# haoheliu/AudioLDM2

Hardware: NVIDIA H100
Metric: 10s clips/sec @200 DDIM steps (audioldm2-full) (higher is better)
Workload: dtype f16x2 (split-fp16 tensor-core operands: weights hi + lo, activations hi + lo in the convolutions and one plane on the token side; fp32 accumulate, fp32 residual stream)

## Files before the change

### audioldm2_b200/csrc/attention.cu

```cuda
#include <float.h>
#include <stdlib.h>

#include "common.cuh"

namespace aldm {

static constexpr int ATT_D = 32;

__device__ __forceinline__ float ex2_approx(float x) {
  float y;
  asm("ex2.approx.ftz.f32 %0, %1;" : "=f"(y) : "f"(x));
  return y;
}

__device__ __forceinline__ void store_out_row(const aldm_attn_desc& d, long long orow, int h, const float* o) {
  aldm_plane_t* hp = reinterpret_cast<aldm_plane_t*>(d.out_hi) + orow * d.ldo + h * ATT_D;
  aldm_plane_t* lp = d.out_lo ? reinterpret_cast<aldm_plane_t*>(d.out_lo) + orow * d.ldo + h * ATT_D : nullptr;
#pragma unroll
  for (int i = 0; i < ATT_D; i += 8) {
    uint4 hh, ll;
    split8(o + i, hh, ll);
    *reinterpret_cast<uint4*>(hp + i) = hh;
    if (lp) *reinterpret_cast<uint4*>(lp + i) = ll;
  }
}

namespace atc {
constexpr int QT = 128, KT = 64, NS = 4;
constexpr int QA = 0;
constexpr int KB = QA + QT * 128;
constexpr int VT = KB + NS * KT * 128;
constexpr int BAR = VT + NS * ATT_D * 128;
constexpr int SMEM = BAR + 128 + 1024;
}

__device__ __forceinline__ uint32_t pack_half2(float a, float b) {
  const __half2 h = __floats2half2_rn(a, b);
  return *reinterpret_cast<const uint32_t*>(&h);
}

__global__ void __launch_bounds__(288, 2) attention_tc_kernel(const __grid_constant__ aldm_attn_desc d) {
  using namespace atc;
  extern __shared__ uint8_t smem_raw[];
  const uint32_t raw = smem_u32(smem_raw);
  const uint32_t base = (raw + 1023u) & ~1023u;
  const uint32_t bar = base + BAR;
  const uint32_t q_full = bar, kv_full0 = bar + 8, kv_empty0 = kv_full0 + 8 * NS;
  const int tid = threadIdx.x, warp = tid >> 5, lane = tid & 31;
  const int b = blockIdx.z, h = blockIdx.y, q0 = blockIdx.x * QT;
  const int bkv = d.kv_bmod > 0 ? b % d.kv_bmod : b;
  const int nt = (d.Nk + KT - 1) / KT;

  if (tid == 0) {
    mbar_init(q_full, 32);
    for (int i = 0; i < NS; ++i) { mbar_init(kv_full0 + 8 * i, 32); mbar_init(kv_empty0 + 8 * i, 8); }
    fence_barrier_init();
  }
  __syncthreads();
  pdl_wait();

  if (warp < 8) {
    const int wg = warp >> 2, g = lane >> 2, t = lane & 3;
    const int rloc = wg * 64 + (warp & 3) * 16 + g;
    const float sl2 = d.scale * 1.4426950408889634f;
    const float* mrow = d.mask ? d.mask + (long long)bkv * d.Nk : nullptr;
    const uint64_t dQ = wgmma_desc_sw128(base + QA + wg * 64 * 128);
    float o[16];
#pragma unroll
    for (int i = 0; i < 16; ++i) o[i] = 0.f;
    float mrun[2] = {-INFINITY, -INFINITY}, lrun[2] = {0.f, 0.f};
    mbar_wait(q_full, 0);
    for (int it = 0; it < nt; ++it) {
      const int k0 = it * KT, st = it % NS;
      mbar_wait(kv_full0 + 8 * st, (it / NS) & 1);
      fence_proxy_async();
      float s[32];
#pragma unroll
      for (int i = 0; i < 32; ++i) s[i] = 0.f;
      const uint64_t dK = wgmma_desc_sw128(base + KB + st * (KT * 128));
      wgmma_fence();
#pragma unroll
      for (int ks = 0; ks < 2; ++ks) wgmma_ss<KT>(s, dQ + 2 * ks, dK + 2 * ks, 1);
      wgmma_commit();
      wgmma_wait<0>();
      wgmma_fence_regs<32>(s);
      float mnew[2], corr[2];
      if (k0 + KT <= d.Nk && !mrow) {
#pragma unroll
        for (int hr = 0; hr < 2; ++hr) {
          float tmax = s[2 * hr];
#pragma unroll
          for (int j = 0; j < 8; ++j) tmax = fmaxf(tmax, fmaxf(s[4 * j + 2 * hr], s[4 * j + 2 * hr + 1]));
          tmax = fmaxf(tmax, __shfl_xor_sync(0xffffffffu, tmax, 1));
          tmax = fmaxf(tmax, __shfl_xor_sync(0xffffffffu, tmax, 2));
          mnew[hr] = fmaxf(mrun[hr], tmax * sl2);
          corr[hr] = ex2_approx(mrun[hr] - mnew[hr]);
#pragma unroll
          for (int j = 0; j < 8; ++j)
#pragma unroll
            for (int e = 0; e < 2; ++e) s[4 * j + 2 * hr + e] = ex2_approx(fmaf(s[4 * j + 2 * hr + e], sl2, -mnew[hr]));
        }
      } else {
#pragma unroll
        for (int hr = 0; hr < 2; ++hr) {
          float tmax = -INFINITY;
#pragma unroll
          for (int j = 0; j < 8; ++j)
#pragma unroll
            for (int e = 0; e < 2; ++e) {
              const int key = k0 + 8 * j + 2 * t + e;
              float v = s[4 * j + 2 * hr + e] * sl2;
              if (key >= d.Nk) v = -INFINITY;
              else if (mrow && __ldg(mrow + key) != 1.0f) v = -FLT_MAX;
              s[4 * j + 2 * hr + e] = v;
              tmax = fmaxf(tmax, v);
            }
          tmax = fmaxf(tmax, __shfl_xor_sync(0xffffffffu, tmax, 1));
          tmax = fmaxf(tmax, __shfl_xor_sync(0xffffffffu, tmax, 2));
          mnew[hr] = fmaxf(mrun[hr], tmax);
          corr[hr] = (mrun[hr] == -INFINITY) ? 0.f : ex2_approx(mrun[hr] - mnew[hr]);
#pragma unroll
          for (int j = 0; j < 8; ++j)
#pragma unroll
            for (int e = 0; e < 2; ++e) {
              const float v = s[4 * j + 2 * hr + e];
              s[4 * j + 2 * hr + e] = (v == -INFINITY) ? 0.f : ex2_approx(v - mnew[hr]);
            }
        }
      }
#pragma unroll
      for (int hr = 0; hr < 2; ++hr) {
        float ps = 0.f;
#pragma unroll
        for (int j = 0; j < 8; ++j) ps += s[4 * j + 2 * hr] + s[4 * j + 2 * hr + 1];
        lrun[hr] = lrun[hr] * corr[hr] + ps;
        mrun[hr] = mnew[hr];
#pragma unroll
        for (int j = 0; j < 4; ++j) { o[4 * j + 2 * hr] *= corr[hr]; o[4 * j + 2 * hr + 1] *= corr[hr]; }
      }
      uint32_t pa[4][4];
#pragma unroll
      for (int kc = 0; kc < 4; ++kc) {
        pa[kc][0] = pack_half2(s[8 * kc + 0], s[8 * kc + 1]);
        pa[kc][1] = pack_half2(s[8 * kc + 2], s[8 * kc + 3]);
        pa[kc][2] = pack_half2(s[8 * kc + 4], s[8 * kc + 5]);
        pa[kc][3] = pack_half2(s[8 * kc + 6], s[8 * kc + 7]);
      }
      const uint64_t dV = wgmma_desc_sw128(base + VT + st * (ATT_D * 128));
      wgmma_fence();
#pragma unroll
      for (int kc = 0; kc < 4; ++kc) wgmma_rs<ATT_D>(o, pa[kc], dV + 2 * kc, 1);
      wgmma_commit();
      wgmma_wait<0>();
      wgmma_fence_regs<16>(o);
      __syncwarp();
      if (lane == 0) mbar_arrive(kv_empty0 + 8 * st);
    }
    if (tid == 0) pdl_launch();
#pragma unroll
    for (int hr = 0; hr < 2; ++hr) {
      float l = lrun[hr];
      l += __shfl_xor_sync(0xffffffffu, l, 1);
      l += __shfl_xor_sync(0xffffffffu, l, 2);
      const int q = q0 + rloc + 8 * hr;
      if (q < d.Nq) {
        const float inv = 1.0f / l;
        const long long orow = (long long)b * d.Nq + q;
        aldm_plane_t* hp = reinterpret_cast<aldm_plane_t*>(d.out_hi) + orow * d.ldo + h * ATT_D + 2 * t;
        aldm_plane_t* lp = d.out_lo ? reinterpret_cast<aldm_plane_t*>(d.out_lo) + orow * d.ldo + h * ATT_D + 2 * t : nullptr;
#pragma unroll
        for (int j = 0; j < 4; ++j) {
          uint32_t hh, ll;
          split2(o[4 * j + 2 * hr] * inv, o[4 * j + 2 * hr + 1] * inv, hh, ll);
          *reinterpret_cast<uint32_t*>(hp + 8 * j) = hh;
          if (lp) *reinterpret_cast<uint32_t*>(lp + 8 * j) = ll;
        }
      }
    }
  } else {
    const aldm_plane_t* qh = reinterpret_cast<const aldm_plane_t*>(d.q_hi);
    const aldm_plane_t* kh = reinterpret_cast<const aldm_plane_t*>(d.k_hi);
    const aldm_plane_t* vh = reinterpret_cast<const aldm_plane_t*>(d.vt_hi);
    for (int idx = lane; idx < QT * 4; idx += 32) {
      const int r = idx >> 2, c = idx & 3;
      const bool ok = q0 + r < d.Nq;
      const long long off = ok ? ((long long)b * d.Nq + q0 + r) * d.ldq + d.q_col + h * ATT_D + c * 8 : 0;
      cp_async_16(base + QA + r * 128 + ((uint32_t)(c ^ (r & 7)) << 4), qh + off, ok ? 16u : 0u);
    }
    cp_async_mbar_arrive_noinc(q_full);
    const int ck = lane & 3, rk = lane >> 2;
    const int cv = lane & 7, rv = lane >> 3;
    const aldm_plane_t* kcol = kh + (long long)bkv * d.Nk * d.ldk + d.k_col + h * ATT_D + ck * 8;
    const long long vrow0 = ((long long)(bkv * d.heads + h) * ATT_D + rv) * d.ld_t + cv * 8;
    const long long kstep = 8ll * d.ldk, vstep = 4ll * d.ld_t;
    for (int it = 0, s = 0, ph = 1; it < nt; ++it) {
      const int k0 = it * KT;
      mbar_wait(kv_empty0 + 8 * s, ph);
      const uint32_t kb = base + KB + s * (KT * 128);
      const aldm_plane_t* kp = kcol + (long long)(k0 + rk) * d.ldk;
#pragma unroll
      for (int i = 0; i < KT / 8; ++i) {
        const int r = rk + 8 * i;
        const bool ok = k0 + r < d.Nk;
        cp_async_16(kb + r * 128 + ((uint32_t)(ck ^ (r & 7)) << 4), ok ? kp + i * kstep : kcol, ok ? 16u : 0u);
      }
      const uint32_t vb = base + VT + s * (ATT_D * 128);
      const bool vok = k0 + cv * 8 < d.Nk;
#pragma unroll
      for (int i = 0; i < ATT_D / 4; ++i) {
        const int r = rv + 4 * i;
        const aldm_plane_t* vp = vh + vrow0 + i * vstep + k0;
        cp_async_16(vb + r * 128 + ((uint32_t)(cv ^ (r & 7)) << 4), vok ? vp : vh, vok ? 16u : 0u);
      }
      cp_async_mbar_arrive_noinc(kv_full0 + 8 * s);
      if (++s == NS) { s = 0; ph ^= 1; }
    }
  }
}

template <int NKT>
__global__ void __launch_bounds__(128) attention_short_kernel(const __grid_constant__ aldm_attn_desc d) {
  __shared__ __align__(16) float sk[NKT][ATT_D];
  __shared__ __align__(16) float sv[NKT][ATT_D];
  __shared__ int sstate[NKT];
  const int tid = threadIdx.x;
  const int b = blockIdx.z, h = blockIdx.y;
  const int bkv = d.kv_bmod > 0 ? b % d.kv_bmod : b;
  pdl_wait();
  {
    const aldm_plane_t* kh = reinterpret_cast<const aldm_plane_t*>(d.k_hi);
    const aldm_plane_t* vh = reinterpret_cast<const aldm_plane_t*>(d.vt_hi);
    for (int idx = tid; idx < NKT * ATT_D; idx += 128) {
      const int key = idx / ATT_D, dim = idx % ATT_D;
      float kv = 0.f, vv = 0.f;
      if (key < d.Nk) {
        const long long ki = ((long long)bkv * d.Nk + key) * d.ldk + d.k_col + h * ATT_D + dim;
        const long long vi = ((long long)(bkv * d.heads + h) * ATT_D + dim) * d.ld_t + key;
        kv = plane_to_f(kh[ki]);
        vv = plane_to_f(vh[vi]);
      }
      sk[key][dim] = kv;
      sv[key][dim] = vv;
    }
    if (tid < NKT) sstate[tid] = tid >= d.Nk ? 2 : ((d.mask && __ldg(d.mask + (long long)bkv * d.Nk + tid) != 1.0f) ? 1 : 0);
  }
  __syncthreads();
  pdl_launch();
  const int q = blockIdx.x * 128 + tid;
  if (q >= d.Nq) return;
  float qv[ATT_D];
  {
    const long long qi = ((long long)b * d.Nq + q) * d.ldq + d.q_col + h * ATT_D;
    const uint4* ph = reinterpret_cast<const uint4*>(reinterpret_cast<const aldm_plane_t*>(d.q_hi) + qi);
#pragma unroll
    for (int c = 0; c < 4; ++c) {
      const uint4 a = __ldg(ph + c);
      const uint32_t aw[4] = {a.x, a.y, a.z, a.w};
#pragma unroll
      for (int e = 0; e < 4; ++e) {
        const float2 f = unpack2(aw[e]);
        qv[c * 8 + 2 * e] = f.x;
        qv[c * 8 + 2 * e + 1] = f.y;
      }
    }
  }
  const float sl2 = d.scale * 1.4426950408889634f;
  float sc[NKT];
  float mx = -INFINITY;
#pragma unroll
  for (int k = 0; k < NKT; ++k) {
    float acc = 0.f;
#pragma unroll
    for (int dd = 0; dd < ATT_D; dd += 4) {
      const float4 kk = *reinterpret_cast<const float4*>(&sk[k][dd]);
      acc = fmaf(qv[dd], kk.x, acc); acc = fmaf(qv[dd + 1], kk.y, acc);
      acc = fmaf(qv[dd + 2], kk.z, acc); acc = fmaf(qv[dd + 3], kk.w, acc);
    }
    const int st = sstate[k];
    const float v = st == 0 ? acc * sl2 : (st == 1 ? -FLT_MAX : -INFINITY);
    sc[k] = v;
    mx = fmaxf(mx, v);
  }
  float l = 0.f;
#pragma unroll
  for (int k = 0; k < NKT; ++k) {
    const float pk = sc[k] == -INFINITY ? 0.f : ex2_approx(sc[k] - mx);
    sc[k] = pk;
    l += pk;
  }
  float o[ATT_D];
#pragma unroll
  for (int i = 0; i < ATT_D; ++i) o[i] = 0.f;
#pragma unroll
  for (int k = 0; k < NKT; ++k) {
#pragma unroll
    for (int dd = 0; dd < ATT_D; dd += 4) {
      const float4 vv = *reinterpret_cast<const float4*>(&sv[k][dd]);
      o[dd] = fmaf(sc[k], vv.x, o[dd]); o[dd + 1] = fmaf(sc[k], vv.y, o[dd + 1]);
      o[dd + 2] = fmaf(sc[k], vv.z, o[dd + 2]); o[dd + 3] = fmaf(sc[k], vv.w, o[dd + 3]);
    }
  }
  const float inv = 1.0f / l;
#pragma unroll
  for (int i = 0; i < ATT_D; ++i) o[i] *= inv;
  store_out_row(d, (long long)b * d.Nq + q, h, o);
}

__global__ void __launch_bounds__(128) attention_simt_kernel(const __grid_constant__ aldm_attn_desc d) {
  const int b = blockIdx.z, h = blockIdx.y;
  const int qi = blockIdx.x * blockDim.x + threadIdx.x;
  if (qi >= d.Nq) return;
  const int bkv = d.kv_bmod > 0 ? b % d.kv_bmod : b;
  auto ld = [](const void* hi, const void* , long long i) {
    return plane_to_f(reinterpret_cast<const aldm_plane_t*>(hi)[i]);
  };
  float q[ATT_D], o[ATT_D];
  for (int i = 0; i < ATT_D; ++i) {
    q[i] = ld(d.q_hi, d.q_lo, ((long long)b * d.Nq + qi) * d.ldq + d.q_col + h * ATT_D + i) * d.scale;
    o[i] = 0.f;
  }
  float mrun = -INFINITY, lrun = 0.f;
  for (int k = 0; k < d.Nk; ++k) {
    float s = 0.f;
    const long long kr = ((long long)bkv * d.Nk + k) * d.ldk + d.k_col + h * ATT_D;
    for (int i = 0; i < ATT_D; ++i) s = fmaf(q[i], ld(d.k_hi, d.k_lo, kr + i), s);
    if (d.mask && d.mask[(long long)bkv * d.Nk + k] != 1.0f) s = -FLT_MAX;
    const float mnew = fmaxf(mrun, s);
    const float corr = (mrun == -INFINITY) ? 0.f : expf(mrun - mnew);
    const float p = expf(s - mnew);
    lrun = lrun * corr + p;
    for (int i = 0; i < ATT_D; ++i)
      o[i] = o[i] * corr + p * ld(d.vt_hi, d.vt_lo, ((long long)(bkv * d.heads + h) * ATT_D + i) * d.ld_t + k);
    mrun = mnew;
  }
  for (int i = 0; i < ATT_D; ++i) o[i] /= lrun;
  store_out_row(d, (long long)b * d.Nq + qi, h, o);
}

int attention_launch(const aldm_attn_desc& d, cudaStream_t st) {
  ALDM_REQUIRE(d.q_hi && d.k_hi && d.vt_hi && d.out_hi, ALDM_E_ARG, "attention: null pointer");
  ALDM_REQUIRE(d.B > 0 && d.heads > 0 && d.Nq > 0 && d.Nk > 0, ALDM_E_SHAPE, "attention: B=%d heads=%d Nq=%d Nk=%d", d.B,
               d.heads, d.Nq, d.Nk);
  ALDM_REQUIRE(d.ldq % 8 == 0 && d.ldk % 8 == 0 && d.ld_t % 8 == 0 && d.ldo % 8 == 0 && d.q_col % 8 == 0 && d.k_col % 8 == 0,
               ALDM_E_ALIGN, "attention: leading dims / column offsets must be multiples of 8");
  ALDM_REQUIRE(d.ld_t >= d.Nk, ALDM_E_SHAPE, "attention: ld_t=%d < Nk=%d", d.ld_t, d.Nk);
  ALDM_REQUIRE(aligned16(d.q_hi) && aligned16(d.k_hi) && aligned16(d.vt_hi) && aligned16(d.out_hi) && aligned16(d.out_lo),
               ALDM_E_ALIGN, "attention: pointers must be 16B aligned");
  ALDM_REQUIRE(d.heads <= 65535 && d.B <= 65535, ALDM_E_SHAPE, "attention: grid too large");
  if (d.impl == ALDM_GEMM_SIMT) {
    dim3 grid(cdiv(d.Nq, 128), d.heads, d.B);
    attention_simt_kernel<<<grid, 128, 0, st>>>(d);
  } else if (d.Nk <= 32 && !(getenv("ALDM_ATTN_SHORT") && getenv("ALDM_ATTN_SHORT")[0] == '0')) {
    dim3 grid(cdiv(d.Nq, 128), d.heads, d.B);
    if (d.Nk <= 8) ALDM_CHECK_CUDA(launch_pdl(attention_short_kernel<8>, grid, dim3(128), 0, st, d));
    else if (d.Nk <= 16) ALDM_CHECK_CUDA(launch_pdl(attention_short_kernel<16>, grid, dim3(128), 0, st, d));
    else ALDM_CHECK_CUDA(launch_pdl(attention_short_kernel<32>, grid, dim3(128), 0, st, d));
  } else {
    static bool configured = false;
    if (!configured) {
      ALDM_CHECK_CUDA(cudaFuncSetAttribute(attention_tc_kernel, cudaFuncAttributeMaxDynamicSharedMemorySize, atc::SMEM));
      configured = true;
    }
    dim3 grid(cdiv(d.Nq, atc::QT), d.heads, d.B);
    ALDM_CHECK_CUDA(launch_pdl(attention_tc_kernel, grid, dim3(288), atc::SMEM, st, d));
  }
  ALDM_CHECK_CUDA(cudaGetLastError());
  return ALDM_OK;
}

__global__ void softmax_rows_kernel(const float* __restrict__ x, int n, float scale, aldm_plane_t* __restrict__ hi,
                                    aldm_plane_t* __restrict__ lo) {
  __shared__ float red[32];
  const long long row = blockIdx.x;
  const float* xp = x + row * n;
  float mx = -INFINITY;
  for (int i = threadIdx.x; i < n; i += blockDim.x) mx = fmaxf(mx, xp[i] * scale);
  for (int o = 16; o > 0; o >>= 1) mx = fmaxf(mx, __shfl_xor_sync(0xffffffffu, mx, o));
  if ((threadIdx.x & 31) == 0) red[threadIdx.x >> 5] = mx;
  __syncthreads();
  mx = red[0];
  for (int w = 1; w < (blockDim.x >> 5); ++w) mx = fmaxf(mx, red[w]);
  __syncthreads();
  float s = 0.f;
  for (int i = threadIdx.x; i < n; i += blockDim.x) s += expf(xp[i] * scale - mx);
  for (int o = 16; o > 0; o >>= 1) s += __shfl_xor_sync(0xffffffffu, s, o);
  if ((threadIdx.x & 31) == 0) red[threadIdx.x >> 5] = s;
  __syncthreads();
  s = 0.f;
  for (int w = 0; w < (blockDim.x >> 5); ++w) s += red[w];
  const float inv = 1.0f / s;
  for (int i = threadIdx.x * 2; i < n; i += blockDim.x * 2) {
    const float a = expf(xp[i] * scale - mx) * inv;
    const float b = (i + 1 < n) ? expf(xp[i + 1] * scale - mx) * inv : 0.f;
    uint32_t h, l;
    split2(a, b, h, l);
    if (i + 1 < n) {
      *reinterpret_cast<uint32_t*>(hi + row * n + i) = h;
      if (lo) *reinterpret_cast<uint32_t*>(lo + row * n + i) = l;
    } else {
      store_split1(hi, lo, row * n + i, a);
    }
  }
}

}

extern "C" int aldm_attention(const aldm_attn_desc* d, void* stream) {
  if (!d) { aldm::set_error("aldm_attention: null desc"); return ALDM_E_ARG; }
  return aldm::attention_launch(*d, reinterpret_cast<cudaStream_t>(stream));
}

extern "C" int aldm_softmax_rows(const float* x, int32_t rows, int32_t n, float scale, void* out_hi, void* out_lo,
                                 void* stream) {
  using namespace aldm;
  ALDM_REQUIRE(x && out_hi && rows > 0 && n > 0, ALDM_E_ARG, "softmax_rows: bad arguments");
  ALDM_REQUIRE(n % 2 == 0, ALDM_E_UNSUPPORTED, "softmax_rows: n must be even");
  softmax_rows_kernel<<<rows, 256, 0, reinterpret_cast<cudaStream_t>(stream)>>>(
      x, n, scale, reinterpret_cast<aldm_plane_t*>(out_hi), reinterpret_cast<aldm_plane_t*>(out_lo));
  ALDM_CHECK_CUDA(cudaGetLastError());
  return ALDM_OK;
}
```

Before: 1.852.

## Pipeline QK and PV wgmma in attention, add lazy rescale and small-Nq config

Restructures the tensor-core attention loop so the QK^T wgmma for the next key tile is issued together with the PV wgmma of the current tile, and softmax runs while PV is in flight. Adds conditional rescaling: the running max is only raised when it grows by more than a threshold, so the output rescale is skipped warp-wide when no row changed. Adds a compile-time PLAIN variant with no mask or tail handling, and a one-warpgroup config for small Nq. This trades more register pressure and extra template instantiations for fewer serialized tensor-core waits. The lazy max also lets exponent values exceed 1 by up to 2^8, which adds fp16 range risk in P.

```diff
diff --git a/audioldm2_b200/csrc/attention.cu b/audioldm2_b200/csrc/attention.cu
--- a/audioldm2_b200/csrc/attention.cu
+++ b/audioldm2_b200/csrc/attention.cu
@@ -26,12 +26,19 @@
 }
 
 namespace atc {
-constexpr int QT = 128, KT = 64, NS = 4;
-constexpr int QA = 0;
-constexpr int KB = QA + QT * 128;
-constexpr int VT = KB + NS * KT * 128;
-constexpr int BAR = VT + NS * ATT_D * 128;
-constexpr int SMEM = BAR + 128 + 1024;
+constexpr int KT = 64, NS = 4;
+constexpr float TAU = 8.f;
+template <int NWG>
+struct Cfg {
+  static constexpr int QT = 64 * NWG;
+  static constexpr int THREADS = 128 * NWG + 32;
+  static constexpr int QA = 0;
+  static constexpr int KB = QA + QT * 128;
+  static constexpr int VT = KB + NS * KT * 128;
+  static constexpr int BAR = VT + NS * ATT_D * 128;
+  static constexpr int SMEM = BAR + 128 + 1024;
+  static constexpr int MIN_CTAS = NWG == 2 ? 2 : 3;
+};
 }
 
 __device__ __forceinline__ uint32_t pack_half2(float a, float b) {
@@ -39,123 +46,174 @@
   return *reinterpret_cast<const uint32_t*>(&h);
 }
 
-__global__ void __launch_bounds__(288, 2) attention_tc_kernel(const __grid_constant__ aldm_attn_desc d) {
+__device__ __forceinline__ void fence_regs_u32(uint32_t (&a)[4][4]) {
+#pragma unroll
+  for (int i = 0; i < 4; ++i)
+#pragma unroll
+    for (int j = 0; j < 4; ++j) asm volatile("" : "+r"(a[i][j])::"memory");
+}
+
+template <bool PLAIN>
+__device__ __forceinline__ void softmax_tile(float (&s)[32], int k0, int t, int Nk, const float* mrow, float sl2,
+                                             float (&mrun)[2], float (&lrun)[2], float (&corr)[2]) {
   using namespace atc;
+  const bool plain = PLAIN || (k0 + KT <= Nk && !mrow);
+  uint32_t out = 0, off = 0;
+  if (!plain) {
+#pragma unroll
+    for (int i = 0; i < 16; ++i) {
+      const int key = k0 + 8 * (i >> 1) + 2 * t + (i & 1);
+      if (key >= Nk) out |= 1u << i;
+      else if (mrow && __ldg(mrow + key) != 1.0f) off |= 1u << i;
+    }
+  }
+  float tmax[2];
+#pragma unroll
+  for (int hr = 0; hr < 2; ++hr) {
+    float m = -INFINITY;
+    if (plain) {
+#pragma unroll
+      for (int j = 0; j < 8; ++j) m = fmaxf(m, fmaxf(s[4 * j + 2 * hr], s[4 * j + 2 * hr + 1]));
+    } else {
+#pragma unroll
+      for (int j = 0; j < 8; ++j)
+#pragma unroll
+        for (int e = 0; e < 2; ++e) {
+          const uint32_t bit = 1u << (2 * j + e);
+          float v = s[4 * j + 2 * hr + e] * sl2;
+          if (out & bit) v = -INFINITY;
+          else if (off & bit) v = -FLT_MAX;
+          s[4 * j + 2 * hr + e] = v;
+          m = fmaxf(m, v);
+        }
+    }
+    m = fmaxf(m, __shfl_xor_sync(0xffffffffu, m, 1));
+    m = fmaxf(m, __shfl_xor_sync(0xffffffffu, m, 2));
+    tmax[hr] = plain ? m * sl2 : m;
+  }
+#pragma unroll
+  for (int hr = 0; hr < 2; ++hr) {
+    corr[hr] = 1.f;
+    if (tmax[hr] > mrun[hr] + TAU) {
+      corr[hr] = ex2_approx(mrun[hr] - tmax[hr]);
+      mrun[hr] = tmax[hr];
+    }
+    const float m = mrun[hr];
+    float ps = 0.f;
+    if (plain) {
+#pragma unroll
+      for (int j = 0; j < 8; ++j)
+#pragma unroll
+        for (int e = 0; e < 2; ++e) {
+          float& v = s[4 * j + 2 * hr + e];
+          v = ex2_approx(fmaf(v, sl2, -m));
+          ps += v;
+        }
+    } else {
+#pragma unroll
+      for (int j = 0; j < 8; ++j)
+#pragma unroll
+        for (int e = 0; e < 2; ++e) {
+          float& v = s[4 * j + 2 * hr + e];
+          v = v == -INFINITY ? 0.f : ex2_approx(v - m);
+          ps += v;
+        }
+    }
+    lrun[hr] = lrun[hr] * corr[hr] + ps;
+  }
+}
+
+__device__ __forceinline__ void pack_p(const float (&s)[32], uint32_t (&pa)[4][4]) {
+#pragma unroll
+  for (int kc = 0; kc < 4; ++kc)
+#pragma unroll
+    for (int i = 0; i < 4; ++i) pa[kc][i] = pack_half2(s[8 * kc + 2 * i], s[8 * kc + 2 * i + 1]);
+}
+
+template <int NWG, bool PLAIN>
+__global__ void __launch_bounds__(atc::Cfg<NWG>::THREADS, atc::Cfg<NWG>::MIN_CTAS) attention_tc_kernel(
+    const __grid_constant__ aldm_attn_desc d) {
+  using namespace atc;
+  using C = Cfg<NWG>;
   extern __shared__ uint8_t smem_raw[];
   const uint32_t raw = smem_u32(smem_raw);
   const uint32_t base = (raw + 1023u) & ~1023u;
-  const uint32_t bar = base + BAR;
+  const uint32_t bar = base + C::BAR;
   const uint32_t q_full = bar, kv_full0 = bar + 8, kv_empty0 = kv_full0 + 8 * NS;
   const int tid = threadIdx.x, warp = tid >> 5, lane = tid & 31;
-  const int b = blockIdx.z, h = blockIdx.y, q0 = blockIdx.x * QT;
+  const int b = blockIdx.z, h = blockIdx.y, q0 = blockIdx.x * C::QT;
   const int bkv = d.kv_bmod > 0 ? b % d.kv_bmod : b;
   const int nt = (d.Nk + KT - 1) / KT;
 
   if (tid == 0) {
     mbar_init(q_full, 32);
-    for (int i = 0; i < NS; ++i) { mbar_init(kv_full0 + 8 * i, 32); mbar_init(kv_empty0 + 8 * i, 8); }
+    for (int i = 0; i < NS; ++i) { mbar_init(kv_full0 + 8 * i, 32); mbar_init(kv_empty0 + 8 * i, 4 * NWG); }
     fence_barrier_init();
   }
   __syncthreads();
   pdl_wait();
 
-  if (warp < 8) {
+  if (warp < 4 * NWG) {
     const int wg = warp >> 2, g = lane >> 2, t = lane & 3;
     const int rloc = wg * 64 + (warp & 3) * 16 + g;
     const float sl2 = d.scale * 1.4426950408889634f;
     const float* mrow = d.mask ? d.mask + (long long)bkv * d.Nk : nullptr;
-    const uint64_t dQ = wgmma_desc_sw128(base + QA + wg * 64 * 128);
+    const uint64_t dQ = wgmma_desc_sw128(base + C::QA + wg * 64 * 128);
     float o[16];
 #pragma unroll
     for (int i = 0; i < 16; ++i) o[i] = 0.f;
-    float mrun[2] = {-INFINITY, -INFINITY}, lrun[2] = {0.f, 0.f};
-    mbar_wait(q_full, 0);
-    for (int it = 0; it < nt; ++it) {
-      const int k0 = it * KT, st = it % NS;
-      mbar_wait(kv_full0 + 8 * st, (it / NS) & 1);
-      fence_proxy_async();
-      float s[32];
-#pragma unroll
-      for (int i = 0; i < 32; ++i) s[i] = 0.f;
-      const uint64_t dK = wgmma_desc_sw128(base + KB + st * (KT * 128));
-      wgmma_fence();
-#pragma unroll
-      for (int ks = 0; ks < 2; ++ks) wgmma_ss<KT>(s, dQ + 2 * ks, dK + 2 * ks, 1);
+    float mrun[2] = {-INFINITY, -INFINITY}, lrun[2] = {0.f, 0.f}, corr[2];
+    float s[32];
+    uint32_t pa[4][4];
+    auto issue_s = [&](int st) {
+      const uint64_t dK = wgmma_desc_sw128(base + C::KB + st * (KT * 128));
+#pragma unroll
+      for (int ks = 0; ks < 2; ++ks) wgmma_ss<KT>(s, dQ + 2 * ks, dK + 2 * ks, ks);
       wgmma_commit();
-      wgmma_wait<0>();
-      wgmma_fence_regs<32>(s);
-      float mnew[2], corr[2];
-      if (k0 + KT <= d.Nk && !mrow) {
-#pragma unroll
-        for (int hr = 0; hr < 2; ++hr) {
-          float tmax = s[2 * hr];
-#pragma unroll
-          for (int j = 0; j < 8; ++j) tmax = fmaxf(tmax, fmaxf(s[4 * j + 2 * hr], s[4 * j + 2 * hr + 1]));
-          tmax = fmaxf(tmax, __shfl_xor_sync(0xffffffffu, tmax, 1));
-          tmax = fmaxf(tmax, __shfl_xor_sync(0xffffffffu, tmax, 2));
-          mnew[hr] = fmaxf(mrun[hr], tmax * sl2);
-          corr[hr] = ex2_approx(mrun[hr] - mnew[hr]);
-#pragma unroll
-          for (int j = 0; j < 8; ++j)
-#pragma unroll
-            for (int e = 0; e < 2; ++e) s[4 * j + 2 * hr + e] = ex2_approx(fmaf(s[4 * j + 2 * hr + e], sl2, -mnew[hr]));
-        }
-      } else {
-#pragma unroll
-        for (int hr = 0; hr < 2; ++hr) {
-          float tmax = -INFINITY;
-#pragma unroll
-          for (int j = 0; j < 8; ++j)
-#pragma unroll
-            for (int e = 0; e < 2; ++e) {
-              const int key = k0 + 8 * j + 2 * t + e;
-              float v = s[4 * j + 2 * hr + e] * sl2;
-              if (key >= d.Nk) v = -INFINITY;
-              else if (mrow && __ldg(mrow + key) != 1.0f) v = -FLT_MAX;
-              s[4 * j + 2 * hr + e] = v;
-              tmax = fmaxf(tmax, v);
-            }
-          tmax = fmaxf(tmax, __shfl_xor_sync(0xffffffffu, tmax, 1));
-          tmax = fmaxf(tmax, __shfl_xor_sync(0xffffffffu, tmax, 2));
-          mnew[hr] = fmaxf(mrun[hr], tmax);
-          corr[hr] = (mrun[hr] == -INFINITY) ? 0.f : ex2_approx(mrun[hr] - mnew[hr]);
-#pragma unroll
-          for (int j = 0; j < 8; ++j)
-#pragma unroll
-            for (int e = 0; e < 2; ++e) {
-              const float v = s[4 * j + 2 * hr + e];
-              s[4 * j + 2 * hr + e] = (v == -INFINITY) ? 0.f : ex2_approx(v - mnew[hr]);
-            }
-        }
-      }
-#pragma unroll
-      for (int hr = 0; hr < 2; ++hr) {
-        float ps = 0.f;
-#pragma unroll
-        for (int j = 0; j < 8; ++j) ps += s[4 * j + 2 * hr] + s[4 * j + 2 * hr + 1];
-        lrun[hr] = lrun[hr] * corr[hr] + ps;
-        mrun[hr] = mnew[hr];
-#pragma unroll
-        for (int j = 0; j < 4; ++j) { o[4 * j + 2 * hr] *= corr[hr]; o[4 * j + 2 * hr + 1] *= corr[hr]; }
-      }
-      uint32_t pa[4][4];
-#pragma unroll
-      for (int kc = 0; kc < 4; ++kc) {
-        pa[kc][0] = pack_half2(s[8 * kc + 0], s[8 * kc + 1]);
-        pa[kc][1] = pack_half2(s[8 * kc + 2], s[8 * kc + 3]);
-        pa[kc][2] = pack_half2(s[8 * kc + 4], s[8 * kc + 5]);
-        pa[kc][3] = pack_half2(s[8 * kc + 6], s[8 * kc + 7]);
-      }
-      const uint64_t dV = wgmma_desc_sw128(base + VT + st * (ATT_D * 128));
-      wgmma_fence();
+    };
+    auto issue_pv = [&](int st) {
+      const uint64_t dV = wgmma_desc_sw128(base + C::VT + st * (ATT_D * 128));
 #pragma unroll
       for (int kc = 0; kc < 4; ++kc) wgmma_rs<ATT_D>(o, pa[kc], dV + 2 * kc, 1);
       wgmma_commit();
+    };
+    mbar_wait(q_full, 0);
+    mbar_wait(kv_full0, 0);
+    fence_proxy_async();
+    wgmma_fence();
+    issue_s(0);
+    wgmma_wait<0>();
+    wgmma_fence_regs<32>(s);
+    softmax_tile<PLAIN>(s, 0, t, d.Nk, mrow, sl2, mrun, lrun, corr);
+    pack_p(s, pa);
+    for (int it = 0; it + 1 < nt; ++it) {
+      const int st = it % NS, st1 = (it + 1) % NS;
+      mbar_wait(kv_full0 + 8 * st1, ((it + 1) / NS) & 1);
+      fence_proxy_async();
+      wgmma_fence();
+      issue_s(st1);
+      issue_pv(st);
+      wgmma_wait<1>();
+      wgmma_fence_regs<32>(s);
+      softmax_tile<PLAIN>(s, (it + 1) * KT, t, d.Nk, mrow, sl2, mrun, lrun, corr);
       wgmma_wait<0>();
       wgmma_fence_regs<16>(o);
+      fence_regs_u32(pa);
       __syncwarp();
       if (lane == 0) mbar_arrive(kv_empty0 + 8 * st);
-    }
+      if (__any_sync(0xffffffffu, corr[0] != 1.f || corr[1] != 1.f)) {
+#pragma unroll
+        for (int hr = 0; hr < 2; ++hr)
+#pragma unroll
+          for (int j = 0; j < 4; ++j) { o[4 * j + 2 * hr] *= corr[hr]; o[4 * j + 2 * hr + 1] *= corr[hr]; }
+      }
+      pack_p(s, pa);
+    }
+    wgmma_fence();
+    issue_pv((nt - 1) % NS);
+    wgmma_wait<0>();
+    wgmma_fence_regs<16>(o);
+    fence_regs_u32(pa);
     if (tid == 0) pdl_launch();
 #pragma unroll
     for (int hr = 0; hr < 2; ++hr) {
@@ -181,11 +239,11 @@
     const aldm_plane_t* qh = reinterpret_cast<const aldm_plane_t*>(d.q_hi);
     const aldm_plane_t* kh = reinterpret_cast<const aldm_plane_t*>(d.k_hi);
     const aldm_plane_t* vh = reinterpret_cast<const aldm_plane_t*>(d.vt_hi);
-    for (int idx = lane; idx < QT * 4; idx += 32) {
+    for (int idx = lane; idx < C::QT * 4; idx += 32) {
       const int r = idx >> 2, c = idx & 3;
       const bool ok = q0 + r < d.Nq;
       const long long off = ok ? ((long long)b * d.Nq + q0 + r) * d.ldq + d.q_col + h * ATT_D + c * 8 : 0;
-      cp_async_16(base + QA + r * 128 + ((uint32_t)(c ^ (r & 7)) << 4), qh + off, ok ? 16u : 0u);
+      cp_async_16(base + C::QA + r * 128 + ((uint32_t)(c ^ (r & 7)) << 4), qh + off, ok ? 16u : 0u);
     }
     cp_async_mbar_arrive_noinc(q_full);
     const int ck = lane & 3, rk = lane >> 2;
@@ -196,7 +254,7 @@
     for (int it = 0, s = 0, ph = 1; it < nt; ++it) {
       const int k0 = it * KT;
       mbar_wait(kv_empty0 + 8 * s, ph);
-      const uint32_t kb = base + KB + s * (KT * 128);
+      const uint32_t kb = base + C::KB + s * (KT * 128);
       const aldm_plane_t* kp = kcol + (long long)(k0 + rk) * d.ldk;
 #pragma unroll
       for (int i = 0; i < KT / 8; ++i) {
@@ -204,7 +262,7 @@
         const bool ok = k0 + r < d.Nk;
         cp_async_16(kb + r * 128 + ((uint32_t)(ck ^ (r & 7)) << 4), ok ? kp + i * kstep : kcol, ok ? 16u : 0u);
       }
-      const uint32_t vb = base + VT + s * (ATT_D * 128);
+      const uint32_t vb = base + C::VT + s * (ATT_D * 128);
       const bool vok = k0 + cv * 8 < d.Nk;
 #pragma unroll
       for (int i = 0; i < ATT_D / 4; ++i) {
@@ -337,6 +395,25 @@
   store_out_row(d, (long long)b * d.Nq + qi, h, o);
 }
 
+template <int NWG, bool PLAIN>
+static cudaError_t attention_tc_launch(const aldm_attn_desc& d, cudaStream_t st) {
+  using C = atc::Cfg<NWG>;
+  static bool configured = false;
+  if (!configured) {
+    const cudaError_t e =
+        cudaFuncSetAttribute(attention_tc_kernel<NWG, PLAIN>, cudaFuncAttributeMaxDynamicSharedMemorySize, C::SMEM);
+    if (e != cudaSuccess) return e;
+    configured = true;
+  }
+  dim3 grid(cdiv(d.Nq, C::QT), d.heads, d.B);
+  return launch_pdl(attention_tc_kernel<NWG, PLAIN>, grid, dim3(C::THREADS), C::SMEM, st, d);
+}
+
+template <int NWG>
+static cudaError_t attention_tc_launch(const aldm_attn_desc& d, cudaStream_t st) {
+  return !d.mask && d.Nk % atc::KT == 0 ? attention_tc_launch<NWG, true>(d, st) : attention_tc_launch<NWG, false>(d, st);
+}
+
 int attention_launch(const aldm_attn_desc& d, cudaStream_t st) {
   ALDM_REQUIRE(d.q_hi && d.k_hi && d.vt_hi && d.out_hi, ALDM_E_ARG, "attention: null pointer");
   ALDM_REQUIRE(d.B > 0 && d.heads > 0 && d.Nq > 0 && d.Nk > 0, ALDM_E_SHAPE, "attention: B=%d heads=%d Nq=%d Nk=%d", d.B,
@@ -355,14 +432,10 @@
     if (d.Nk <= 8) ALDM_CHECK_CUDA(launch_pdl(attention_short_kernel<8>, grid, dim3(128), 0, st, d));
     else if (d.Nk <= 16) ALDM_CHECK_CUDA(launch_pdl(attention_short_kernel<16>, grid, dim3(128), 0, st, d));
     else ALDM_CHECK_CUDA(launch_pdl(attention_short_kernel<32>, grid, dim3(128), 0, st, d));
+  } else if (d.Nq <= 64) {
+    ALDM_CHECK_CUDA(attention_tc_launch<1>(d, st));
   } else {
-    static bool configured = false;
-    if (!configured) {
-      ALDM_CHECK_CUDA(cudaFuncSetAttribute(attention_tc_kernel, cudaFuncAttributeMaxDynamicSharedMemorySize, atc::SMEM));
-      configured = true;
-    }
-    dim3 grid(cdiv(d.Nq, atc::QT), d.heads, d.B);
-    ALDM_CHECK_CUDA(launch_pdl(attention_tc_kernel, grid, dim3(288), atc::SMEM, st, d));
+    ALDM_CHECK_CUDA(attention_tc_launch<2>(d, st));
   }
   ALDM_CHECK_CUDA(cudaGetLastError());
   return ALDM_OK;
```

Result: faster. 1.881, median of 6 (+1.6%).
